# fenghansen/PNNP

Hardware: AMD Instinct MI355X
Metric: 512x512x4 raw crops/sec (train step) (higher is better)
Workload: dtype f32 (operands, accumulation and results; 3x3 and ConvTranspose2d / 1x1 / stride-2 forward / backward-data / backward-weight multiply on the fp16 matrix cores through a per-tensor-scaled 2-way split, 22 significand bits per operand: csrc/h2.h); 1 GPU; PNNP noise-proxy ('pr' physics sampler, SonyA7S2 params) + UNetSeeInDark nf=32 train step (fwd + L1 + bwd + Adam); crops_per_gpu=16, global_batch=16, crop=4x512x512, parallelism=dp1, optimizer=Adam lr 1e-4

## Files before the change

pnnp_amd/csrc/wgrad_h2s.hip:

```cpp
#include "h2.h"
#include "wgrad_s.h"

typedef _Float16 f16x8 __attribute__((ext_vector_type(8)));

namespace {

#ifndef WHS_G_AUX
#define WHS_G_AUX 2
#endif
#ifndef WHS_ROLL
#define WHS_ROLL 1
#endif
struct Wh2s {
    static constexpr int PIECES = 2, MFMAS = 3, G_AUX = WHS_G_AUX;
    static constexpr bool SCALED = true, ROLL = WHS_ROLL;
    static constexpr bool MW2 = true;
    static constexpr int TH22 = 2, TH21 = 3, TH12 = 3, TH11 = 4;
    static constexpr int pa(int G) { return G == 1 ? 1 : 0; }
    static constexpr int pb(int G) { return G == 0 ? 1 : 0; }
    static __device__ __forceinline__ f32x16 mfma(u32x4 a, u32x4 b, f32x16 c) {
        return __builtin_amdgcn_mfma_f32_32x32x16_f16(__builtin_bit_cast(f16x8, a), __builtin_bit_cast(f16x8, b), c, 0, 0, 0);
    }
    static __device__ __forceinline__ void scale_exps(const WsArgs& a, int& se_g, int& se_x) {
        unsigned axb = a.amax_x[0] ? a.amax_x[0][0] : 0u;
        if (a.amax_x[1]) { const unsigned a2 = a.amax_x[1][0]; axb = a2 > axb ? a2 : axb; }
        se_x = __builtin_amdgcn_readfirstlane(pnnp_h2_scale_exp(axb));
        se_g = __builtin_amdgcn_readfirstlane(a.amax_g ? pnnp_h2_scale_exp(a.amax_g[0]) : 0);
    }
    static __device__ __forceinline__ float unscale(float v, int dexp) { return __builtin_ldexpf(v, dexp); }
    static __device__ __forceinline__ void split(f32x4 v, float sc, unsigned (&p)[2][2]) {
        split_h2(v.x, v.y, sc, p[0][0], p[1][0]);
        split_h2(v.z, v.w, sc, p[0][1], p[1][1]);
    }
};

}

int pnnp_wh2s_th(int M, int N) { return ws_th<Wh2s>(M, N); }
int pnnp_wh2s_launch(const WsArgs& a, hipStream_t s) { return ws_launch<Wh2s>(a, s); }
```

pnnp_amd/csrc/wgrad_s.h:

```cpp
#pragma once
#include "common.h"

struct WsArgs {
    const float* G; int Gcs;
    const float* X[2]; int Xcs[2];
    int n_split;
    int B, H, W, M, N;
    float* slab;
    float* bias_slab;
    int Z;
    const unsigned* amax_g; const unsigned* amax_x[2];
};
int pnnp_wx3s_launch(const WsArgs& a, hipStream_t s);
int pnnp_wx3s_th(int M, int N);
int pnnp_wh2s_launch(const WsArgs& a, hipStream_t s);
int pnnp_wh2s_th(int M, int N);

#ifndef WX3_ALT_SIGN
#define WX3_ALT_SIGN 1
#endif

namespace {

constexpr int NCW = 12, NPW = 4, NTHR = 64 * (NCW + NPW);
constexpr int XC = 34;
constexpr unsigned OOB = 0x80000000u;
#define WS_BARRIER() asm volatile("s_waitcnt lgkmcnt(0)\n\ts_barrier" ::: "memory")
#ifdef WHS_STAMPS
#define WS_T(v) { const long long now_ = clock64(); v += now_ - tlast_; tlast_ = now_; }
#else
#define WS_T(v)
#endif

template <class Scheme, int MO, int NO, int TH, int MW = 1> struct WsCfg {
    static constexpr int P = Scheme::PIECES;
    static constexpr int WK = 4 * MW / (MO * NO);
    static constexpr int KS = TH * 2, KSW = KS / WK;
    static constexpr int GPIX = TH * 32, XPIX = (TH + 2) * XC;
    static constexpr int G_BYTES = MO * P * GPIX * 64, X_BYTES = NO * P * XPIX * 64, IMG_BYTES = G_BYTES + X_BYTES, LDS_BYTES = 2 * IMG_BYTES;
    static constexpr int GT = 256 / MO, XT = 256 / NO;
    static constexpr int NG = GPIX * 8 / GT, NX = (XPIX * 8 + XT - 1) / XT;
    static_assert(MO * NO * WK == 4 * MW && KSW * WK == KS && (MW == 1 || MW == MO), "wave layout");
    static_assert((GPIX * 8) % GT == 0, "G slots divide evenly (the bias sums count every pixel once)");
    static_assert(LDS_BYTES <= 160 * 1024 && LDS_BYTES >= NCW * 16 * 64 * 4, "LDS budget (images; the final reduction aliases them, one accumulator block at a time)");
};

template <class Scheme, int MO, int NO, int TH, int MW>
__global__ void __launch_bounds__(NTHR, 1)
wgrad_s_kernel(const WsArgs a) {
    using Cfg = WsCfg<Scheme, MO, NO, TH, MW>;
    constexpr int P = Cfg::P, WK = Cfg::WK, KSW = Cfg::KSW, GPIX = Cfg::GPIX, XPIX = Cfg::XPIX, G_BYTES = Cfg::G_BYTES, IMG_BYTES = Cfg::IMG_BYTES, NG = Cfg::NG, NX = Cfg::NX;
    extern __shared__ __attribute__((aligned(16))) char smem[];
    const int tid = threadIdx.x, lane = tid & 63;
    const int wave = __builtin_amdgcn_readfirstlane(tid >> 6);

    int se_g = 0, se_x = 0;
    if constexpr (Scheme::SCALED) Scheme::scale_exps(a, se_g, se_x);
    const int n_tiles = a.N / (32 * NO);
    int id = blockIdx.x;
    const int z = id % a.Z; id /= a.Z;
    const int ni = id % n_tiles, mi = id / n_tiles;
    const int m0 = mi * 32 * MO, n0 = ni * 32 * NO;
    const int tiles_x = (a.W + 31) >> 5, tiles_y = (a.H + TH - 1) / TH;
    const int ntile = tiles_x * tiles_y * a.B;
    if (z >= ntile) return;

    if (wave >= NCW) {
        const int pw = wave - NCW;
        const int q8 = lane & 7;
        const int gblk = MO == 2 ? pw >> 1 : 0, lg = MO == 2 ? (pw & 1) * 64 + lane : pw * 64 + lane;
        const int xblk = NO == 2 ? pw >> 1 : 0, lx = NO == 2 ? (pw & 1) * 64 + lane : pw * 64 + lane;
        constexpr int GSTEP = Cfg::GT / 8;
        const int gp0 = lg >> 3;
        const unsigned g_base = (unsigned)(gp0 * a.Gcs + q8 * 4) * 4u;
        const int g_dst0 = (gblk * P * GPIX + gp0) * 64 + q8 * 8;
        const int xd = (n0 + 32 * xblk >= a.n_split) ? 1 : 0;
        const int xch0 = n0 + 32 * xblk - (xd ? a.n_split : 0);
        const int xcs = a.Xcs[xd];
        int x_rc[NX];
#pragma unroll
        for (int k = 0; k < NX; ++k) {
            int j = lx + Cfg::XT * k;
            if (j >= XPIX * 8) j -= Cfg::XT;
            const int pix = j >> 3;
            const int r = pix / XC;
            x_rc[k] = (r << 8) | (pix - r * XC);
        }
        const __amdgpu_buffer_rsrc_t rsg = __builtin_amdgcn_make_buffer_rsrc((void*)(a.G + m0 + 32 * gblk), 0, 0x7fffffff, 0x00020000);
        const int xshift = (a.W + 1) * xcs;
        const __amdgpu_buffer_rsrc_t rsx = __builtin_amdgcn_make_buffer_rsrc((void*)(a.X[xd] + xch0 - xshift), 0, 0x7fffffff, 0x00020000);
        f32x4 rg[NG], rx[NX];
        float bsum[4] = {0.f, 0.f, 0.f, 0.f};
        const float sgs = __uint_as_float(((unsigned)(se_g + 127) << 23) | ((Scheme::SCALED && WX3_ALT_SIGN && (z & 1)) ? 0x80000000u : 0u));
        const float sxs = __uint_as_float((unsigned)(se_x + 127) << 23);
        const unsigned sflip = (!Scheme::SCALED && WX3_ALT_SIGN && (z & 1)) ? 0x80000000u : 0u;
        struct TileSc { int gso, xso, rlim, clim, y0, x0; };
        auto tile_sc = [&](int tile) {
            int q = tile;
            const int tx = q % tiles_x; q /= tiles_x;
            const int ty = q % tiles_y;
            const int b = q / tiles_y;
            TileSc t;
            t.x0 = tx * 32; t.y0 = ty * TH;
            t.gso = (((b * a.H + t.y0) * a.W) + t.x0) * a.Gcs * 4;
            t.xso = ((((b * a.H + t.y0 - 1) * a.W) + t.x0 - 1) * xcs + xshift) * 4;
            t.rlim = a.H - t.y0; t.clim = a.W - t.x0;
            return t;
        };
        auto load_g = [&](auto ktag, const TileSc& t) {
            constexpr int k = decltype(ktag)::value;
            const int gr = (GSTEP * k) >> 5, gc = gp0 + ((GSTEP * k) & 31);
            const int bad = (t.rlim - 1 - gr) | (t.clim - 1 - gc);
            rg[k] = __builtin_bit_cast(f32x4, __builtin_amdgcn_raw_buffer_load_b128(rsg, bad < 0 ? OOB : g_base, t.gso + (gr * a.W + ((GSTEP * k) & 31)) * a.Gcs * 4, Scheme::G_AUX));
        };
        auto load_x = [&](auto ktag, const TileSc& t) {
            constexpr int k = decltype(ktag)::value;
            const int xr = x_rc[k] >> 8, xc = x_rc[k] & 255;
            const int yy = t.y0 - 1 + xr, xx = t.x0 - 1 + xc;
            const int bad = yy | (a.H - 1 - yy) | xx | (a.W - 1 - xx);
            rx[k] = __builtin_bit_cast(f32x4, __builtin_amdgcn_raw_buffer_load_b128(rsx, bad < 0 ? OOB : (unsigned)((xr * a.W + xc) * xcs + q8 * 4) * 4u, t.xso, 0));
        };
        auto load_tile = [&](int tile) {
            const TileSc t = tile_sc(tile);
            static_for<0, NG>([&](auto kt) { load_g(kt, t); });
            static_for<0, NX>([&](auto kt) { load_x(kt, t); });
        };
        auto stage = [&](f32x4 v, float sc, char* ib, int dst, int pstride) {
            unsigned pc[P][2];
            Scheme::split(v, sc, pc);
#pragma unroll
            for (int p = 0; p < P; ++p) *reinterpret_cast<u32x2*>(ib + dst + p * pstride) = u32x2{pc[p][0], pc[p][1]};
        };
        auto stage_g = [&](auto ktag, char* ib) {
            constexpr int k = decltype(ktag)::value;
            f32x4 v = rg[k];
            bsum[0] += v.x; bsum[1] += v.y; bsum[2] += v.z; bsum[3] += v.w;
            if constexpr (!Scheme::SCALED)
                v = f32x4{__uint_as_float(__float_as_uint(v.x) ^ sflip), __uint_as_float(__float_as_uint(v.y) ^ sflip),
                          __uint_as_float(__float_as_uint(v.z) ^ sflip), __uint_as_float(__float_as_uint(v.w) ^ sflip)};
            stage(v, sgs, ib, g_dst0 + GSTEP * k * 64, GPIX * 64);
        };
        auto stage_x = [&](auto ktag, char* ib) {
            constexpr int k = decltype(ktag)::value;
            stage(rx[k], sxs, ib, G_BYTES + (xblk * P * XPIX + (x_rc[k] >> 8) * XC + (x_rc[k] & 255)) * 64 + q8 * 8, XPIX * 64);
        };
        auto stage_tile = [&](int img) {
            char* ib = smem + img * IMG_BYTES;
            static_for<0, NG>([&](auto kt) { stage_g(kt, ib); });
            static_for<0, NX>([&](auto kt) { stage_x(kt, ib); });
        };
        auto roll_tile = [&](int img, int tile_after) {
            char* ib = smem + img * IMG_BYTES;
            const TileSc t = tile_sc(tile_after);
            static_for<0, NG>([&](auto kt) { stage_g(kt, ib); load_g(kt, t); __builtin_amdgcn_sched_barrier(0); });
            static_for<0, NX>([&](auto kt) { stage_x(kt, ib); load_x(kt, t); __builtin_amdgcn_sched_barrier(0); });
        };
        load_tile(z);
        stage_tile(0);
        if (z + a.Z < ntile) load_tile(z + a.Z);
        int img = 0;
#ifdef WHS_STAMPS
        long long t_stage = 0, t_issue = 0, t_bar = 0, tlast_ = clock64(), tall = tlast_; int ntl = 0;
#endif
        for (int tile = z; tile < ntile; tile += a.Z) {
            WS_BARRIER();
            WS_T(t_bar)
#ifdef WHS_STAMPS
            ++ntl;
#endif
            if (Scheme::ROLL && tile + 2 * a.Z < ntile) {
                roll_tile(img ^ 1, tile + 2 * a.Z);
                WS_T(t_stage)
            } else if (tile + a.Z < ntile) {
                stage_tile(img ^ 1);
                WS_T(t_stage)
                if (tile + 2 * a.Z < ntile) load_tile(tile + 2 * a.Z);
                WS_T(t_issue)
            }
            img ^= 1;
        }
#ifdef WHS_STAMPS
        if (lane == 0) {
            float* d = a.slab + ((int64_t)blockIdx.x * (NCW + NPW) + wave) * 8;
            d[0] = (float)t_stage; d[1] = (float)t_issue; d[2] = (float)t_bar; d[4] = (float)(clock64() - tall); d[5] = (float)ntl;
        }
#endif
        if (WK > 1) {
#pragma unroll
            for (int i = 0; i < 6 * MW; ++i) WS_BARRIER();
        }
        WS_BARRIER();
        constexpr int NSLOTS = Cfg::GT / 8;
        if (a.bias_slab && ni == 0) {
            float* bs = reinterpret_cast<float*>(smem);
            const int slot = lg >> 3;
#pragma unroll
            for (int c = 0; c < 4; ++c) bs[((gblk * 8 + q8) * 4 + c) * NSLOTS + slot] = bsum[c];
        }
        WS_BARRIER();
        if (a.bias_slab && ni == 0 && pw < 1 && lane < 32 * MO) {
            float* bs = reinterpret_cast<float*>(smem);
            const int b2 = lane >> 5, ch = lane & 31;
            float s = 0.f;
            for (int k = 0; k < NSLOTS; ++k) s += bs[((b2 * 8 + (ch >> 2)) * 4 + (ch & 3)) * NSLOTS + k];
            a.bias_slab[(int64_t)z * a.M + m0 + b2 * 32 + ch] = (WX3_ALT_SIGN && (z & 1)) ? -s : s;
        }
        return;
    }

    const int tr = wave % 3, rest = wave / 3;
    const int wk = rest % WK, no = (rest / WK) % NO, mo = MW == 1 ? rest / (WK * NO) : 0;
    const int l31 = lane & 31, half = lane >> 5;
    f32x16 acc[MW][3];
#pragma unroll
    for (int mb = 0; mb < MW; ++mb)
#pragma unroll
        for (int t = 0; t < 3; ++t)
#pragma unroll
            for (int r = 0; r < 16; ++r) acc[mb][t][r] = 0.f;
    const int tr_lane = ((8 * (lane >> 5) + ((lane & 15) >> 2)) * 64) + (16 * ((lane >> 4) & 1) + 4 * (lane & 3)) * 2;
    auto tr_read = [&](const char* base) {
        const s16x4 lo = __builtin_amdgcn_ds_read_tr16_b64_v4i16((__attribute__((address_space(3))) s16x4*)(base));
        const s16x4 hi = __builtin_amdgcn_ds_read_tr16_b64_v4i16((__attribute__((address_space(3))) s16x4*)(base + 4 * 64));
        const u32x2 a0 = __builtin_bit_cast(u32x2, lo), a1 = __builtin_bit_cast(u32x2, hi);
        return u32x4{a0.x, a0.y, a1.x, a1.y};
    };
    int img = 0;
#ifdef WHS_STAMPS
    long long t_mfma = 0, t_bar = 0, tlast_ = clock64(), tall = tlast_; int ntl = 0;
    const long long t_entry = tlast_;
    long long t_first = 0;
#endif
    for (int tile = z; tile < ntile; tile += a.Z) {
        WS_BARRIER();
        WS_T(t_bar)
#ifdef WHS_STAMPS
        if (!ntl) t_first = tlast_ - t_entry;
        ++ntl;
#endif
        const char* gimg = smem + img * IMG_BYTES;
        const char* ximg = gimg + G_BYTES;
        constexpr int NBUF = MW == 1 ? 2 : 1;
        u32x4 av[NBUF][MW][P], bv[NBUF][P];
        auto gload = [&](int kl, u32x4 (&ax)[MW][P]) {
            const int ks = wk * KSW + kl;
#pragma unroll
            for (int mb = 0; mb < MW; ++mb) {
                const char* gbase = gimg + (((mo + mb) * P) * GPIX + (ks >> 1) * 32 + (ks & 1) * 16) * 64 + tr_lane;
#pragma unroll
                for (int p = 0; p < P; ++p) ax[mb][p] = tr_read(gbase + p * GPIX * 64);
            }
        };
        auto xload = [&](int kl, int dx, u32x4 (&bx)[P]) {
            const int ks = wk * KSW + kl;
            const char* xbase = ximg + ((no * P) * XPIX + ((ks >> 1) + tr) * XC + (ks & 1) * 16 + dx) * 64 + tr_lane;
#pragma unroll
            for (int p = 0; p < P; ++p) bx[p] = tr_read(xbase + p * XPIX * 64);
        };
        gload(0, av[0]);
        xload(0, 0, bv[0]);
#pragma unroll
        for (int kl = 0; kl < KSW; ++kl) {
#pragma unroll
            for (int dx = 0; dx < 3; ++dx) {
                const int s = kl * 3 + dx;
                if constexpr (NBUF == 2) {
                    if (s + 1 < KSW * 3) xload((s + 1) / 3, (s + 1) % 3, bv[(s + 1) & 1]);
                    if (dx == 2 && kl + 1 < KSW) gload(kl + 1, av[(kl + 1) & 1]);
                    __builtin_amdgcn_sched_barrier(0);
                }
                const u32x4 (&ax)[MW][P] = av[NBUF == 2 ? (kl & 1) : 0];
                const u32x4 (&bx)[P] = bv[NBUF == 2 ? (s & 1) : 0];
#pragma unroll
                for (int mb = 0; mb < MW; ++mb)
#pragma unroll
                    for (int G = 0; G < Scheme::MFMAS; ++G) acc[mb][dx] = Scheme::mfma(ax[mb][Scheme::pa(G)], bx[Scheme::pb(G)], acc[mb][dx]);
                __builtin_amdgcn_sched_barrier(0);
                if constexpr (NBUF == 1) {
                    if (s + 1 < KSW * 3) xload((s + 1) / 3, (s + 1) % 3, bv[0]);
                    if (dx == 2 && kl + 1 < KSW) gload(kl + 1, av[0]);
                    __builtin_amdgcn_sched_barrier(0);
                }
            }
        }
        img ^= 1;
#ifdef WHS_STAMPS
        __builtin_amdgcn_sched_barrier(0);
        asm volatile("s_nop 0" ::: "memory");
#endif
        WS_T(t_mfma)
    }
#ifdef WHS_STAMPS
    const long long t_loop_end = clock64();
#endif
    float* red = reinterpret_cast<float*>(smem);
    const int dexp = -(se_g + se_x);
    float* const slab_z = a.slab + (int64_t)z * a.M * a.N * 9;
#pragma unroll
    for (int mb = 0; mb < MW; ++mb)
#pragma unroll
    for (int dx = 0; dx < 3; ++dx) {
        f32x16 v = acc[mb][dx];
        const int t = tr * 3 + dx;
        if constexpr (WK > 1) {
            WS_BARRIER();
#pragma unroll
            for (int r = 0; r < 16; ++r) red[(wave * 16 + r) * 64 + lane] = v[r];
            WS_BARRIER();
            if (wk == 0) {
                const int c4 = (lane & 7) * 4;
                const unsigned n_u = (unsigned)a.N;
                const unsigned base = (unsigned)((t * a.M + m0 + (mo + mb) * 32) * a.N + n0 + no * 32 + c4);
#pragma unroll
                for (int i = 0; i < 4; ++i) {
                    const int row = (lane >> 3) + 8 * i;
                    const int r = ((row >> 3) << 2) | (row & 3), hf = (row >> 2) & 1;
                    f32x4 sum = {0.f, 0.f, 0.f, 0.f};
#pragma unroll
                    for (int k = 0; k < WK; ++k) sum += *reinterpret_cast<const f32x4*>(red + ((wave + 3 * k) * 16 + r) * 64 + hf * 32 + c4);
#pragma unroll
                    for (int c = 0; c < 4; ++c) sum[c] = Scheme::unscale(sum[c], dexp);
                    *reinterpret_cast<f32x4*>(slab_z + base + (unsigned)row * n_u) = sum;
                }
            }
        } else if (wk == 0) {
            const unsigned base = (unsigned)((t * a.M + m0 + (mo + mb) * 32 + 4 * half) * a.N + n0 + no * 32 + l31);
            const unsigned n_u = (unsigned)a.N;
#pragma unroll
            for (int r = 0; r < 16; ++r) slab_z[base + (unsigned)((r & 3) + 8 * (r >> 2)) * n_u] = Scheme::unscale(v[r], dexp);
        }
    }
    WS_BARRIER();
    WS_BARRIER();
#ifdef WHS_STAMPS
    __builtin_amdgcn_s_waitcnt(0x0f70);
    if (lane == 0) {
        float* d = a.slab + ((int64_t)blockIdx.x * (NCW + NPW) + wave) * 8;
        d[0] = (float)t_mfma; d[1] = (float)t_first; d[2] = (float)t_bar; d[3] = (float)(clock64() - t_loop_end); d[4] = (float)(t_loop_end - tall); d[5] = (float)ntl;
    }
#endif
}

template <class Scheme, int MO, int NO, int TH, int MW = 1>
int ws_launch_tile(const WsArgs& a, hipStream_t s) {
    using Cfg = WsCfg<Scheme, MO, NO, TH, MW>;
    auto kern = wgrad_s_kernel<Scheme, MO, NO, TH, MW>;
    static PnnpPerDevice lds_once;
    if (pnnp_allow_lds(lds_once, kern, Cfg::LDS_BYTES) != PNNP_OK) return PNNP_E_LAUNCH;
    const int blocks = (a.M / (32 * MO)) * (a.N / (32 * NO)) * a.Z;
    hipLaunchKernelGGL(kern, dim3(blocks), dim3(NTHR), Cfg::LDS_BYTES, s, a);
    return pnnp_launch_status();
}

template <class Scheme>
int ws_th(int M, int N) { return (M % 64 == 0) ? ((N % 64 == 0) ? Scheme::TH22 : Scheme::TH21) : ((N % 64 == 0) ? Scheme::TH12 : Scheme::TH11); }

template <class Scheme>
int ws_launch(const WsArgs& a, hipStream_t s) {
    if ((int64_t)a.M * a.N * 9 >= (1ll << 31)) return PNNP_E_UNSUPPORTED;
    if (a.M % 64 == 0) return a.N % 64 == 0 ? ws_launch_tile<Scheme, 2, 2, Scheme::TH22, Scheme::MW2 ? 2 : 1>(a, s) : ws_launch_tile<Scheme, 2, 1, Scheme::TH21>(a, s);
    return a.N % 64 == 0 ? ws_launch_tile<Scheme, 1, 2, Scheme::TH12>(a, s) : ws_launch_tile<Scheme, 1, 1, Scheme::TH11>(a, s);
}

}
```

pnnp_amd/csrc/wgrad_x3s.hip:

```cpp
#include "x3.h"
#include "wgrad_s.h"

typedef __bf16 bf16x8 __attribute__((ext_vector_type(8)));

namespace {

struct Wx3s {
    static constexpr int PIECES = 3, MFMAS = 6;
    static constexpr bool SCALED = false, ROLL = false;
    static constexpr int G_AUX = 0;
    static constexpr bool MW2 = false;
    static constexpr int TH22 = 2, TH21 = 3, TH12 = 2, TH11 = 4;
    static constexpr int pa(int G) { return G == 0 ? 0 : (G == 1 ? 2 : (G == 2 ? 1 : (G == 3 ? 0 : (G == 4 ? 1 : 0)))); }
    static constexpr int pb(int G) { return G == 0 ? 2 : (G == 1 ? 0 : (G == 2 ? 1 : (G == 3 ? 1 : (G == 4 ? 0 : 0)))); }
    static __device__ __forceinline__ f32x16 mfma(u32x4 a, u32x4 b, f32x16 c) {
        return __builtin_amdgcn_mfma_f32_32x32x16_bf16(__builtin_bit_cast(bf16x8, a), __builtin_bit_cast(bf16x8, b), c, 0, 0, 0);
    }
    static __device__ __forceinline__ float unscale(float v, int) { return v; }
    static __device__ __forceinline__ void split(f32x4 v, float, unsigned (&p)[3][2]) {
        split2(v.x, v.y, p[0][0], p[1][0], p[2][0]);
        split2(v.z, v.w, p[0][1], p[1][1], p[2][1]);
    }
};

}

int pnnp_wx3s_th(int M, int N) { return ws_th<Wx3s>(M, N); }
int pnnp_wx3s_launch(const WsArgs& a, hipStream_t s) { return ws_launch<Wx3s>(a, s); }
```

Before: 1103 crops/s.

## Assign contiguous vertical tile runs per block and optionally reuse halo rows in LDS

The weight-gradient kernel now gives each block a contiguous range of tiles, ordered so consecutive tiles are vertically adjacent. This should improve L2 locality of the overlapping input halo rows. An optional window mode copies the two shared halo rows from the previous LDS image instead of reloading them from global memory. The window mode is gated behind per-scheme flags that default to off, so by default only the reordering and contiguous scheduling take effect. It adds extra LDS traffic and branching when enabled.

After: 1104 crops/s (median of 6 runs). Within noise of the previous version (+0.1%).

```diff
diff --git a/pnnp_amd/csrc/wgrad_h2s.hip b/pnnp_amd/csrc/wgrad_h2s.hip
--- a/pnnp_amd/csrc/wgrad_h2s.hip
+++ b/pnnp_amd/csrc/wgrad_h2s.hip
@@ -11,11 +11,15 @@
 #ifndef WHS_ROLL
 #define WHS_ROLL 1
 #endif
+#ifndef WHS_WIN
+#define WHS_WIN 0
+#endif
 struct Wh2s {
     static constexpr int PIECES = 2, MFMAS = 3, G_AUX = WHS_G_AUX;
     static constexpr bool SCALED = true, ROLL = WHS_ROLL;
     static constexpr bool MW2 = true;
     static constexpr int TH22 = 2, TH21 = 3, TH12 = 3, TH11 = 4;
+    static constexpr bool WIN22 = WHS_WIN & 1, WIN21 = WHS_WIN & 2, WIN12 = WHS_WIN & 4, WIN11 = WHS_WIN & 8;
     static constexpr int pa(int G) { return G == 1 ? 1 : 0; }
     static constexpr int pb(int G) { return G == 0 ? 1 : 0; }
     static __device__ __forceinline__ f32x16 mfma(u32x4 a, u32x4 b, f32x16 c) {
diff --git a/pnnp_amd/csrc/wgrad_s.h b/pnnp_amd/csrc/wgrad_s.h
--- a/pnnp_amd/csrc/wgrad_s.h
+++ b/pnnp_amd/csrc/wgrad_s.h
@@ -16,6 +16,9 @@
 int pnnp_wh2s_launch(const WsArgs& a, hipStream_t s);
 int pnnp_wh2s_th(int M, int N);
 
+#ifndef WS_WINDOW
+#define WS_WINDOW 1
+#endif
 #ifndef WX3_ALT_SIGN
 #define WX3_ALT_SIGN 1
 #endif
@@ -40,6 +43,11 @@
     static constexpr int G_BYTES = MO * P * GPIX * 64, X_BYTES = NO * P * XPIX * 64, IMG_BYTES = G_BYTES + X_BYTES, LDS_BYTES = 2 * IMG_BYTES;
     static constexpr int GT = 256 / MO, XT = 256 / NO;
     static constexpr int NG = GPIX * 8 / GT, NX = (XPIX * 8 + XT - 1) / XT;
+    static constexpr bool WIN = WS_WINDOW && (MO == 2 ? (NO == 2 ? Scheme::WIN22 : Scheme::WIN21) : (NO == 2 ? Scheme::WIN12 : Scheme::WIN11));
+    static constexpr int xclass(int k) {
+        const int pmin = (XT * ((k == NX - 1 && k > 0) ? k - 1 : k)) >> 3, pmax = (XT * k + XT - 1) >> 3;
+        return (!WIN || pmin / XC >= 2) ? 0 : (pmax / XC < 2 ? 2 : 1);
+    }
     static_assert(MO * NO * WK == 4 * MW && KSW * WK == KS && (MW == 1 || MW == MO), "wave layout");
     static_assert((GPIX * 8) % GT == 0, "G slots divide evenly (the bias sums count every pixel once)");
     static_assert(LDS_BYTES <= 160 * 1024 && LDS_BYTES >= NCW * 16 * 64 * 4, "LDS budget (images; the final reduction aliases them, one accumulator block at a time)");
@@ -64,6 +72,7 @@
     const int tiles_x = (a.W + 31) >> 5, tiles_y = (a.H + TH - 1) / TH;
     const int ntile = tiles_x * tiles_y * a.B;
     if (z >= ntile) return;
+    const int lo = (int)((int64_t)z * ntile / a.Z), hi = (int)((int64_t)(z + 1) * ntile / a.Z);
 
     if (wave >= NCW) {
         const int pw = wave - NCW;
@@ -94,13 +103,14 @@
         const float sgs = __uint_as_float(((unsigned)(se_g + 127) << 23) | ((Scheme::SCALED && WX3_ALT_SIGN && (z & 1)) ? 0x80000000u : 0u));
         const float sxs = __uint_as_float((unsigned)(se_x + 127) << 23);
         const unsigned sflip = (!Scheme::SCALED && WX3_ALT_SIGN && (z & 1)) ? 0x80000000u : 0u;
-        struct TileSc { int gso, xso, rlim, clim, y0, x0; };
+        struct TileSc { int gso, xso, rlim, clim, y0, x0, win; };
         auto tile_sc = [&](int tile) {
             int q = tile;
-            const int tx = q % tiles_x; q /= tiles_x;
-            const int ty = q % tiles_y;
-            const int b = q / tiles_y;
+            const int ty = q % tiles_y; q /= tiles_y;
+            const int tx = q % tiles_x;
+            const int b = q / tiles_x;
             TileSc t;
+            t.win = (Cfg::WIN && ty > 0 && tile > lo) ? -1 : 0;
             t.x0 = tx * 32; t.y0 = ty * TH;
             t.gso = (((b * a.H + t.y0) * a.W) + t.x0) * a.Gcs * 4;
             t.xso = ((((b * a.H + t.y0 - 1) * a.W) + t.x0 - 1) * xcs + xshift) * 4;
@@ -117,13 +127,15 @@
             constexpr int k = decltype(ktag)::value;
             const int xr = x_rc[k] >> 8, xc = x_rc[k] & 255;
             const int yy = t.y0 - 1 + xr, xx = t.x0 - 1 + xc;
-            const int bad = yy | (a.H - 1 - yy) | xx | (a.W - 1 - xx);
+            int bad = yy | (a.H - 1 - yy) | xx | (a.W - 1 - xx);
+            if constexpr (Cfg::xclass(k) != 0) bad |= t.win & (xr - 2);
             rx[k] = __builtin_bit_cast(f32x4, __builtin_amdgcn_raw_buffer_load_b128(rsx, bad < 0 ? OOB : (unsigned)((xr * a.W + xc) * xcs + q8 * 4) * 4u, t.xso, 0));
         };
         auto load_tile = [&](int tile) {
             const TileSc t = tile_sc(tile);
             static_for<0, NG>([&](auto kt) { load_g(kt, t); });
             static_for<0, NX>([&](auto kt) { load_x(kt, t); });
+            return t.win;
         };
         auto stage = [&](f32x4 v, float sc, char* ib, int dst, int pstride) {
             unsigned pc[P][2];
@@ -140,41 +152,57 @@
                           __uint_as_float(__float_as_uint(v.z) ^ sflip), __uint_as_float(__float_as_uint(v.w) ^ sflip)};
             stage(v, sgs, ib, g_dst0 + GSTEP * k * 64, GPIX * 64);
         };
-        auto stage_x = [&](auto ktag, char* ib) {
-            constexpr int k = decltype(ktag)::value;
-            stage(rx[k], sxs, ib, G_BYTES + (xblk * P * XPIX + (x_rc[k] >> 8) * XC + (x_rc[k] & 255)) * 64 + q8 * 8, XPIX * 64);
-        };
-        auto stage_tile = [&](int img) {
+        auto stage_x = [&](auto ktag, int img, int win) {
+            constexpr int k = decltype(ktag)::value, cls = Cfg::xclass(k);
+            char* ib = smem + img * IMG_BYTES;
+            const int dst = G_BYTES + (xblk * P * XPIX + (x_rc[k] >> 8) * XC + (x_rc[k] & 255)) * 64 + q8 * 8;
+            bool reuse = false;
+            if constexpr (cls == 2) reuse = win != 0;
+            if constexpr (cls == 1) reuse = (win & ((x_rc[k] >> 8) - 2)) < 0;
+            if (cls != 0 && reuse) {
+                const char* sb = smem + (img ^ 1) * IMG_BYTES + TH * XC * 64;
+                u32x2 w[P];
+#pragma unroll
+                for (int p = 0; p < P; ++p) w[p] = *reinterpret_cast<const u32x2*>(sb + dst + p * XPIX * 64);
+#pragma unroll
+                for (int p = 0; p < P; ++p) *reinterpret_cast<u32x2*>(ib + dst + p * XPIX * 64) = w[p];
+            } else {
+                stage(rx[k], sxs, ib, dst, XPIX * 64);
+            }
+        };
+        auto stage_tile = [&](int img, int win) {
             char* ib = smem + img * IMG_BYTES;
             static_for<0, NG>([&](auto kt) { stage_g(kt, ib); });
-            static_for<0, NX>([&](auto kt) { stage_x(kt, ib); });
-        };
-        auto roll_tile = [&](int img, int tile_after) {
+            static_for<0, NX>([&](auto kt) { stage_x(kt, img, win); });
+        };
+        auto roll_tile = [&](int img, int tile_after, int win) {
             char* ib = smem + img * IMG_BYTES;
             const TileSc t = tile_sc(tile_after);
             static_for<0, NG>([&](auto kt) { stage_g(kt, ib); load_g(kt, t); __builtin_amdgcn_sched_barrier(0); });
-            static_for<0, NX>([&](auto kt) { stage_x(kt, ib); load_x(kt, t); __builtin_amdgcn_sched_barrier(0); });
-        };
-        load_tile(z);
-        stage_tile(0);
-        if (z + a.Z < ntile) load_tile(z + a.Z);
+            static_for<0, NX>([&](auto kt) { stage_x(kt, img, win); load_x(kt, t); __builtin_amdgcn_sched_barrier(0); });
+            return t.win;
+        };
+        load_tile(lo);
+        stage_tile(0, 0);
+        int win = 0;
+        if (lo + 1 < hi) win = load_tile(lo + 1);
         int img = 0;
 #ifdef WHS_STAMPS
         long long t_stage = 0, t_issue = 0, t_bar = 0, tlast_ = clock64(), tall = tlast_; int ntl = 0;
 #endif
-        for (int tile = z; tile < ntile; tile += a.Z) {
+        for (int tile = lo; tile < hi; ++tile) {
             WS_BARRIER();
             WS_T(t_bar)
 #ifdef WHS_STAMPS
             ++ntl;
 #endif
-            if (Scheme::ROLL && tile + 2 * a.Z < ntile) {
-                roll_tile(img ^ 1, tile + 2 * a.Z);
+            if (Scheme::ROLL && tile + 2 < hi) {
+                win = roll_tile(img ^ 1, tile + 2, win);
                 WS_T(t_stage)
-            } else if (tile + a.Z < ntile) {
-                stage_tile(img ^ 1);
+            } else if (tile + 1 < hi) {
+                stage_tile(img ^ 1, win);
                 WS_T(t_stage)
-                if (tile + 2 * a.Z < ntile) load_tile(tile + 2 * a.Z);
+                if (tile + 2 < hi) win = load_tile(tile + 2);
                 WS_T(t_issue)
             }
             img ^= 1;
@@ -231,7 +259,7 @@
     const long long t_entry = tlast_;
     long long t_first = 0;
 #endif
-    for (int tile = z; tile < ntile; tile += a.Z) {
+    for (int tile = lo; tile < hi; ++tile) {
         WS_BARRIER();
         WS_T(t_bar)
 #ifdef WHS_STAMPS
diff --git a/pnnp_amd/csrc/wgrad_x3s.hip b/pnnp_amd/csrc/wgrad_x3s.hip
--- a/pnnp_amd/csrc/wgrad_x3s.hip
+++ b/pnnp_amd/csrc/wgrad_x3s.hip
@@ -5,12 +5,16 @@
 
 namespace {
 
+#ifndef WX3S_WIN
+#define WX3S_WIN 0
+#endif
 struct Wx3s {
     static constexpr int PIECES = 3, MFMAS = 6;
     static constexpr bool SCALED = false, ROLL = false;
     static constexpr int G_AUX = 0;
     static constexpr bool MW2 = false;
     static constexpr int TH22 = 2, TH21 = 3, TH12 = 2, TH11 = 4;
+    static constexpr bool WIN22 = WX3S_WIN & 1, WIN21 = WX3S_WIN & 2, WIN12 = WX3S_WIN & 4, WIN11 = WX3S_WIN & 8;
     static constexpr int pa(int G) { return G == 0 ? 0 : (G == 1 ? 2 : (G == 2 ? 1 : (G == 3 ? 0 : (G == 4 ? 1 : 0)))); }
     static constexpr int pb(int G) { return G == 0 ? 2 : (G == 1 ? 0 : (G == 2 ? 1 : (G == 3 ? 1 : (G == 4 ? 0 : 0)))); }
     static __device__ __forceinline__ f32x16 mfma(u32x4 a, u32x4 b, f32x16 c) {
```
